# Skylarking/MARL

Hardware: NVIDIA B200
Metric: QMIX learner episode-samples/sec (2s3z shape) (higher is better)
Workload: dtype f32

## Files before the change

### marl_b200/csrc/common.cuh

```cuda
#pragma once
#include <cuda_runtime.h>
#include <stdint.h>

#define MARL_H 64
#define MARL_G (3 * MARL_H)

#define MARL_OK 0
#define MARL_EINVAL (-1)

#define MARL_LAUNCH_CHECK()                                   \
    do {                                                      \
        cudaError_t e__ = cudaGetLastError();                 \
        if (e__ != cudaSuccess) return (int)e__;              \
    } while (0)

#include <cstdlib>
#include <utility>

namespace marl {

constexpr int kNumSMs = 148;

__device__ __forceinline__ void pdl_wait() { asm volatile("griddepcontrol.wait;" ::: "memory"); }
__device__ __forceinline__ void pdl_trigger() { asm volatile("griddepcontrol.launch_dependents;" ::: "memory"); }
// ... 22 lines not shown
    return cudaLaunchKernelEx(&cfg, kern, KArgs(std::forward<Args>(args))...);
}
inline int& linear_prio() { static int v = 0; return v; }
struct LinearPrio {
    int keep;
    explicit LinearPrio(int p) : keep(linear_prio()) { linear_prio() = p; }
    ~LinearPrio() { linear_prio() = keep; }
};
template <class... KArgs, class... Args>
inline cudaError_t launch_pdl(void (*kern)(KArgs...), dim3 grid, dim3 block, size_t smem, cudaStream_t st, Args&&... args) {
    return launch_pdl_prio(0, kern, grid, block, smem, st, std::forward<Args>(args)...);
}

__device__ __forceinline__ float warp_sum(float v) {
#pragma unroll
    for (int o = 16; o > 0; o >>= 1) v += __shfl_xor_sync(0xffffffffu, v, o);
    return v;
}

__device__ __forceinline__ void cp_async16(void* smem, const void* gmem) {
    const unsigned s = (unsigned)__cvta_generic_to_shared(smem);
    asm volatile("cp.async.cg.shared.global [%0], [%1], 16;\n" ::"r"(s), "l"(gmem));
}
__device__ __forceinline__ void cp_async_commit() { asm volatile("cp.async.commit_group;\n" ::); }
template <int N>
__device__ __forceinline__ void cp_async_wait() { asm volatile("cp.async.wait_group %0;\n" ::"n"(N)); }

__device__ __forceinline__ float sigmoidf_acc(float x) { return 1.0f / (1.0f + expf(-x)); }

struct LinOperand {
    const float* x;   int ldx;  int K1;
    const float* x2;  int ldx2; int K2;
    int x2_shift;
    int x2_period;
    int onehot_mod;
    long long x_bs, x2_bs;
    int onehot_z;
};

__device__ __forceinline__ float lin_load(const LinOperand& a, int z, int m, int k) {
    if (k < a.K1) return __ldg(a.x + (long long)z * a.x_bs + (long long)m * a.ldx + k);
    k -= a.K1;
    if (k < a.K2) {
        int mm = m;
        if (a.x2_shift) {
            if ((m % a.x2_period) < a.x2_shift) return 0.0f;
// ... 12 lines not shown
```

### marl_b200/csrc/qmix.cu

```cuda
#include "linear.h"
#include "forkjoin.h"
#include "../../include/marl_b200.h"
#include "profile.h"
#include "tgemm.h"

#ifdef MARL_MIX_TRACE
__device__ long long* g_mix_trace_ptr = nullptr;
#define MIX_SEL_STAMP(tag)                                                                                      \
    do {                                                                                                        \
        if (threadIdx.x == 0 && (blockIdx.x == 0 || blockIdx.x == 300) && g_mix_trace_ptr) {                     \
            long long* t__ = g_mix_trace_ptr + (blockIdx.x ? 512 : 0);                                           \
            long long now__; asm volatile("mov.u64 %0, %%globaltimer;" : "=l"(now__));                           \
            const int n__ = (int)t__[510]; if (n__ < 60) { t__[2 * n__] = (tag); t__[2 * n__ + 1] = now__; t__[510] = n__ + 1; } \
        }                                                                                                       \
    } while (0)
#endif
#include "select.cuh"

namespace marl {

constexpr int E = MARL_QMIX_EMBED;
#ifndef MARL_QMIX_WARPS
#define MARL_QMIX_WARPS 8
#endif
constexpr int kQmixWarps = MARL_QMIX_WARPS;
constexpr int kQmixCtasPerSm = 32 / kQmixWarps;
constexpr int kQmixMaxAgents = 64;

enum { QMIX_FWD = 0, QMIX_BWD = 1, QMIX_TD = 2 };

struct QmixMixArgs {
    int M, N, A, mode;
    const float* hy;  const float* q;  const float* wb2;  const float* bb2;
    const float* hy_t; const float* q_t; const float* wb2_t; const float* bb2_t;
    const float* r; const float* term; const float* padded; float gamma;
    const float* dq_tot_in;
    float* q_tot; float* q_tot_t;
    float* dhy;
    float* dq_small;
    const long long* u; float* dq_dense;
    const float* fc2_w; float* dhext;
    SelectArgs sel;
    float* g_wb2; float* g_bb2; float* scalars;
    long long* trace;
};
#ifdef MARL_MIX_TRACE
#define MIX_STAMP(tag) MIX_SEL_STAMP(tag)
#else
#define MIX_STAMP(tag) do { } while (0)
#endif

__device__ __forceinline__ float qmix_forward_lane(const float* __restrict__ y, const float* __restrict__ q, int N,
                                                   float wb2e, float bb2, int lane, float& pre, float& hid,
                                                   float& w2raw, float& hb2) {
    float acc = y[N * E + lane];
#pragma unroll 4
    for (int n = 0; n < N; ++n) acc = fmaf(q[n], fabsf(y[n * E + lane]), acc);
    pre = acc;
    hid = acc > 0.0f ? acc : (expf(acc) - 1.0f);
    w2raw = y[N * E + E + lane];
    hb2 = y[N * E + 2 * E + lane];
    float part = hid * fabsf(w2raw) + fmaxf(hb2, 0.0f) * wb2e;
    return warp_sum(part) + bb2;
}

__global__ void __launch_bounds__(kQmixWarps * 32, kQmixCtasPerSm) qmix_mix_kernel(QmixMixArgs a) {
#ifdef MARL_MIX_TRACE
    if (threadIdx.x == 0 && (blockIdx.x == 0 || blockIdx.x == 300)) g_mix_trace_ptr = a.trace;
#endif
    MIX_STAMP(0);
    pdl_enter();
    MIX_STAMP(1);
    __shared__ float sdq[kQmixWarps][kQmixMaxAgents];
    __shared__ float sred[kQmixWarps][E + 1];
    __shared__ float ssel[kQmixWarps][2][kQmixMaxAgents];
    extern __shared__ __align__(16) float ssel_dyn[];
    const float* heads = nullptr;
    if (a.sel.q && a.sel.heads) {
        const int m_first = blockIdx.x * kQmixWarps + (threadIdx.x >> 5);
        if (m_first < a.M)
            warp_stage_hidden_async(a.sel, m_first, a.N, a.A, threadIdx.x & 31, ssel_dyn + (threadIdx.x >> 5) * select_warp_floats(a.N, a.A, true));
        float* h = ssel_dyn + kQmixWarps * select_warp_floats(a.N, a.A, true);
        stage_heads(a.sel, a.A, h);
        heads = h;
        __syncthreads();
    }
    bool prestaged = a.sel.q && a.sel.heads;
    MIX_STAMP(2);
    const int lane = threadIdx.x & 31, warp = threadIdx.x >> 5;
    const int N = a.N, C = N * E + 3 * E;
    const float wb2e = a.wb2[lane], bb2 = a.bb2[0];
    float wb2te = 0.f, bb2t = 0.f;
    if (a.mode == QMIX_TD) { wb2te = a.wb2_t[lane]; bb2t = a.bb2_t[0]; }
    float acc_wb2 = 0.f, acc_bb2 = 0.f, acc_sq = 0.f, acc_mask = 0.f;
    for (int m = blockIdx.x * kQmixWarps + warp; m < a.M; m += gridDim.x * kQmixWarps) {
        const float* __restrict__ y = a.hy + (long long)m * C;
        const float* q = a.q + (long long)m * N;
        const float* qt = a.q_t + (long long)m * N;
        if (a.sel.q) {
            warp_select(a.sel, m, N, a.A, lane, ssel_dyn + warp * select_warp_floats(N, a.A, a.sel.heads), ssel[warp][0], ssel[warp][1], heads, prestaged);
            prestaged = false;
            q = ssel[warp][0]; qt = ssel[warp][1];
        }
        MIX_STAMP(3);
        float pre, hid, w2raw, hb2;
        const float tot = qmix_forward_lane(y, q, N, wb2e, bb2, lane, pre, hid, w2raw, hb2);
        if (lane == 0 && a.q_tot) a.q_tot[m] = tot;
        MIX_STAMP(4);
        if (a.mode == QMIX_FWD) continue;
        float G;
        if (a.mode == QMIX_TD) {
            float p2, h2, w2t, hbt;
            const float tot_t = qmix_forward_lane(a.hy_t + (long long)m * C, qt, N, wb2te, bb2t,
                                                  lane, p2, h2, w2t, hbt);
            if (lane == 0 && a.q_tot_t) a.q_tot_t[m] = tot_t;
            const float mask = 1.0f - a.padded[m];
            const float yt = a.r[m] + a.gamma * tot_t * (1.0f - a.term[m]);
            const float d = mask * (yt - tot);
            acc_sq += d * d; acc_mask += mask;
            G = -2.0f * mask * d;
        } else {
            G = a.dq_tot_in[m];
        }
        MIX_STAMP(5);
        float* __restrict__ dy = a.dhy + (long long)m * C;
        const float dpre = G * fabsf(w2raw) * (pre > 0.0f ? 1.0f : (hid + 1.0f));
        const float sgn2 = (w2raw > 0.0f) ? 1.0f : (w2raw < 0.0f ? -1.0f : 0.0f);
        dy[N * E + lane] = dpre;
        dy[N * E + E + lane] = G * hid * sgn2;
        dy[N * E + 2 * E + lane] = (hb2 > 0.0f) ? G * wb2e : 0.0f;
        acc_wb2 += G * fmaxf(hb2, 0.0f);
        acc_bb2 += G;
#pragma unroll 4
        for (int n = 0; n < N; ++n) {
            const float w1raw = y[n * E + lane];
            const float sgn1 = (w1raw > 0.0f) ? 1.0f : (w1raw < 0.0f ? -1.0f : 0.0f);
            dy[n * E + lane] = dpre * q[n] * sgn1;
            const float dqn = warp_sum(dpre * fabsf(w1raw));
            if (lane == 0) sdq[warp][n] = dqn;
        }
        __syncwarp();
        MIX_STAMP(6);
        if (a.dq_small)
            for (int n = lane; n < N; n += 32) a.dq_small[(long long)m * N + n] = sdq[warp][n];
        if (a.dq_dense) {
            const int A = a.A;
            for (int i = lane; i < N * A; i += 32) {
                const int n = i / A, c = i - n * A;
                a.dq_dense[(long long)m * N * A + i] = (c == (int)a.u[(long long)m * N + n]) ? sdq[warp][n] : 0.0f;
            }
        }
        if (a.dhext) warp_dhext(a.fc2_w, a.u, m, N, lane, sdq[warp], a.dhext);
        __syncwarp();
        MIX_STAMP(7);
    }
    if (a.mode == QMIX_FWD) return;
    sred[warp][lane] = acc_wb2;
    if (lane == 0) sred[warp][E] = acc_bb2;
    __syncthreads();
    if (warp == 0) {
        float v = 0.f, b = 0.f;
        for (int w = 0; w < kQmixWarps; ++w) { v += sred[w][lane]; b += sred[w][E]; }
        if (a.g_wb2) atomicAdd(a.g_wb2 + lane, v);
        if (lane == 0 && a.g_bb2) atomicAdd(a.g_bb2, b);
    }
    if (a.mode == QMIX_TD) {
        __syncthreads();
        if (lane == 0) { sred[warp][0] = acc_sq; sred[warp][1] = acc_mask; }
        __syncthreads();
        if (threadIdx.x == 0) {
            float v = 0.f, b = 0.f;
            for (int w = 0; w < kQmixWarps; ++w) { v += sred[w][0]; b += sred[w][1]; }
            atomicAdd(a.scalars, v); atomicAdd(a.scalars + 1, b);
        }
    }
    MIX_STAMP(8);
}

static int hyper_fwd(int M, int N, int S, const marl_qmix_params* p, const float* s, float* hy, cudaStream_t st) {
    LinearFwd f{};
    f.in = plain_operand(s, S, S);
    f.w = p->wcat; f.ldw = S; f.bias = p->bcat;
    f.y = hy; f.ldy = N * E + 3 * E; f.M = M; f.N = N * E + 3 * E; f.batch = 1;
    return linear_fwd(f, st);
}

static int hyper_wgrad(int M, int N, int S, const float* s, const float* dhy, const marl_qmix_grads* g, cudaStream_t st) {
    LinearWgrad w{};
    w.dy = dhy; w.lddy = N * E + 3 * E; w.in = plain_operand(s, S, S);
    w.dw = g->wcat; w.ldw = S; w.db = g->bcat; w.M = M; w.N = N * E + 3 * E; w.batch = 1;
    return linear_wgrad(w, st);
}

static int hyper2_fwd(int M, int N, int S, const marl_qmix_hyper2* p, const float* s, float* h, float* hy, cudaStream_t st) {
    const int hh = p->hh, C = N * E + 3 * E;
    int rc;
    LinearFwd f{};
    f.in = plain_operand(s, S, S); f.w = p->w_in; f.ldw = S; f.bias = p->b_in;
    f.y = h; f.ldy = 2 * hh; f.M = M; f.N = 2 * hh; f.relu = 1; f.batch = 1;
// ... 24 lines not shown
    w.dy = dhy + N * E; w.lddy = C; w.in = plain_operand(s, S, S); w.dw = g->w_b1; w.ldw = S; w.db = g->b_b1; w.M = M; w.N = E; w.batch = 1;
    if ((rc = linear_wgrad(w, st))) return rc;
    w.dy = dhy + N * E + 2 * E; w.dw = g->w_b20; w.db = g->b_b20;
    if ((rc = linear_wgrad(w, st))) return rc;
    LinearWgrad o1{};
    o1.dy = dhy; o1.lddy = C; o1.in = plain_operand(h, 2 * hh, hh); o1.dw = g->w1_out; o1.ldw = hh; o1.db = g->b1_out; o1.M = M; o1.N = N * E; o1.batch = 1;
    if ((rc = linear_wgrad(o1, st))) return rc;
    LinearWgrad o2{};
    o2.dy = dhy + N * E + E; o2.lddy = C; o2.in = plain_operand(h + hh, 2 * hh, hh); o2.dw = g->w2_out; o2.ldw = hh; o2.db = g->b2_out; o2.M = M; o2.N = E; o2.batch = 1;
    if ((rc = linear_wgrad(o2, st))) return rc;
    LinearDgrad d1{};
    d1.dy = dhy; d1.lddy = C; d1.w = p->w1_out; d1.ldw = hh; d1.dx = dh; d1.lddx = 2 * hh; d1.relu_src = h; d1.ldrs = 2 * hh;
    d1.M = M; d1.N = N * E; d1.K = hh; d1.batch = 1;
    if ((rc = linear_dgrad(d1, st))) return rc;
    LinearDgrad d2{};
    d2.dy = dhy + N * E + E; d2.lddy = C; d2.w = p->w2_out; d2.ldw = hh; d2.dx = dh + hh; d2.lddx = 2 * hh; d2.relu_src = h + hh; d2.ldrs = 2 * hh;
    d2.M = M; d2.N = E; d2.K = hh; d2.batch = 1;
    if ((rc = linear_dgrad(d2, st))) return rc;
    LinearWgrad i{};
    i.dy = dh; i.lddy = 2 * hh; i.in = plain_operand(s, S, S); i.dw = g->w_in; i.ldw = S; i.db = g->b_in; i.M = M; i.N = 2 * hh; i.batch = 1;
    return linear_wgrad(i, st);
}

static int mix_grid(int M) {
    int blocks = (M + kQmixWarps - 1) / kQmixWarps;
    return blocks < 1 ? 1 : (blocks > kQmixCtasPerSm * kNumSMs ? kQmixCtasPerSm * kNumSMs : blocks);
}

}

using namespace marl;

static bool qmix_params_ok(const marl_qmix_params* p) { return p && p->wcat && p->bcat && p->wb2 && p->bb2; }

extern "C" int marl_qmix_fwd(int M, int N, int S, const marl_qmix_params* p, const float* q, const float* s, float* hy,
                             float* q_tot, void* stream) {
    if (M < 0 || N < 1 || N > kQmixMaxAgents || S < 1 || !qmix_params_ok(p) || !q || !s || !hy || !q_tot) return MARL_EINVAL;
    if (M == 0) return MARL_OK;
    cudaStream_t st = (cudaStream_t)stream;
    int rc = hyper_fwd(M, N, S, p, s, hy, st);
    if (rc) return rc;
    QmixMixArgs a{};
    a.M = M; a.N = N; a.mode = QMIX_FWD; a.hy = hy; a.q = q; a.wb2 = p->wb2; a.bb2 = p->bb2; a.q_tot = q_tot;
    { ProfScope ps_("qmix_mix_kernel", st); launch_pdl(qmix_mix_kernel, dim3(mix_grid(M)), dim3(kQmixWarps * 32), 0, st, a); }
    MARL_LAUNCH_CHECK();
    return MARL_OK;
}

extern "C" int marl_qmix_bwd(int M, int N, int S, const marl_qmix_params* p, const float* q, const float* s,
                             const float* hy, const float* dq_tot, float* dhy, float* dq, const marl_qmix_grads* g,
                             void* stream) {
    if (M < 0 || N < 1 || N > kQmixMaxAgents || S < 1 || !qmix_params_ok(p) || !q || !s || !hy || !dq_tot || !dhy || !g)
        return MARL_EINVAL;
    if (M == 0) return MARL_OK;
    cudaStream_t st = (cudaStream_t)stream;
    QmixMixArgs a{};
    a.M = M; a.N = N; a.mode = QMIX_BWD; a.hy = hy; a.q = q; a.wb2 = p->wb2; a.bb2 = p->bb2;
    a.dq_tot_in = dq_tot; a.dhy = dhy; a.dq_small = dq; a.g_wb2 = g->wb2; a.g_bb2 = g->bb2;
    { ProfScope ps_("qmix_mix_kernel", st); launch_pdl(qmix_mix_kernel, dim3(mix_grid(M)), dim3(kQmixWarps * 32), 0, st, a); }
    MARL_LAUNCH_CHECK();
    return hyper_wgrad(M, N, S, s, dhy, g, st);
}

extern "C" int marl_qmix_td_fwd_bwd(const marl_dims* d, const marl_qmix_params* p, const marl_qmix_params* pt,
                                    const float* s, const float* s_next, float* q_chosen, float* q_tc,
                                    const long long* u, const float* r, const float* terminated, const float* padded,
                                    float gamma, float* hy, float* hy_target, float* dhy, float* q_tot, float* q_tot_target,
                                    float* dq, const marl_qmix_grads* g, float* scalars, int flags, const float* fc2_w,
                                    float* dhext, const marl_select_fused* sel, void* stream) {
    if (!d || !p || !pt || !p->wb2 || !p->bb2 || !pt->wb2 || !pt->bb2 || !s || !s_next || !q_chosen || !q_tc || !r ||
        !terminated || !padded || !hy || !hy_target || !dhy || !g || !scalars)
        return MARL_EINVAL;
    if (!(flags & 1) && (!p->wcat || !p->bcat || !pt->wcat || !pt->bcat)) return MARL_EINVAL;
    if (!(flags & 2) && (!g->wcat || !g->bcat)) return MARL_EINVAL;
    if ((dq || dhext || sel) && !u) return MARL_EINVAL;
    if (sel && !select_ok(sel)) return MARL_EINVAL;
    if (dhext && (!fc2_w || ((uintptr_t)fc2_w & 7) || ((uintptr_t)dhext & 7))) return MARL_EINVAL;
    if (d->N < 1 || d->N > kQmixMaxAgents || d->S < 1) return MARL_EINVAL;
    const int M = d->B * d->L;
    if (M <= 0) return MARL_OK;
    cudaStream_t st = (cudaStream_t)stream;
    pdl_scope((long long)M * d->N);
    int rc;
    if (!(flags & 1)) {
        ForkJoin fj(st, 2);
        if ((rc = hyper_fwd(M, d->N, d->S, p, s, hy, fj.lane(0)))) return rc;
        if ((rc = hyper_fwd(M, d->N, d->S, pt, s_next, hy_target, fj.lane(1)))) return rc;
        fj.join();
    }
    QmixMixArgs a{};
    a.M = M; a.N = d->N; a.A = d->A; a.mode = QMIX_TD;
    a.hy = hy; a.q = q_chosen; a.wb2 = p->wb2; a.bb2 = p->bb2;
    a.hy_t = hy_target; a.q_t = q_tc; a.wb2_t = pt->wb2; a.bb2_t = pt->bb2;
    a.r = r; a.term = terminated; a.padded = padded; a.gamma = gamma;
    a.q_tot = q_tot; a.q_tot_t = q_tot_target; a.dhy = dhy; a.u = u; a.dq_dense = dq;
    a.fc2_w = fc2_w; a.dhext = dhext;
    if (sel) a.sel = select_args(sel, u, q_chosen, q_tc);
    a.g_wb2 = g->wb2; a.g_bb2 = g->bb2; a.scalars = scalars;
    a.trace = trace_buffer();
    const size_t dyn = sel ? select_smem(kQmixWarps, d->N, d->A, sel->hidden_evals != nullptr) : 0;
    if (dyn > kSelectSmemMax) return MARL_EINVAL;
    if (dyn > 40 * 1024) {
        static bool attr_set = false;
        if (!attr_set) { cudaFuncSetAttribute(qmix_mix_kernel, cudaFuncAttributeMaxDynamicSharedMemorySize, (int)kSelectSmemMax); attr_set = true; }
    }
    { ProfScope ps_("qmix_mix_kernel", st); launch_pdl(qmix_mix_kernel, dim3(mix_grid(M)), dim3(kQmixWarps * 32), dyn, st, a); }
    MARL_LAUNCH_CHECK();
    if (flags & 2) return MARL_OK;
    return hyper_wgrad(M, d->N, d->S, s, dhy, g, st);
}

extern "C" int marl_qmix_mix_fwd(int M, int N, const marl_qmix_params* p, const float* q, const float* hy, float* q_tot,
                                 void* stream) {
    if (M < 0 || N < 1 || N > kQmixMaxAgents || !p || !p->wb2 || !p->bb2 || !q || !hy || !q_tot) return MARL_EINVAL;
    if (M == 0) return MARL_OK;
    cudaStream_t st = (cudaStream_t)stream;
    QmixMixArgs a{};
    a.M = M; a.N = N; a.mode = QMIX_FWD; a.hy = hy; a.q = q; a.wb2 = p->wb2; a.bb2 = p->bb2; a.q_tot = q_tot;
    { ProfScope ps_("qmix_mix_kernel", st); launch_pdl(qmix_mix_kernel, dim3(mix_grid(M)), dim3(kQmixWarps * 32), 0, st, a); }
    MARL_LAUNCH_CHECK();
    return MARL_OK;
}

extern "C" int marl_qmix_mix_bwd(int M, int N, const marl_qmix_params* p, const float* q, const float* hy,
                                 const float* dq_tot, float* dhy, float* dq, const marl_qmix_grads* g, void* stream) {
    if (M < 0 || N < 1 || N > kQmixMaxAgents || !p || !p->wb2 || !p->bb2 || !q || !hy || !dq_tot || !dhy || !g) return MARL_EINVAL;
    if (M == 0) return MARL_OK;
    cudaStream_t st = (cudaStream_t)stream;
    QmixMixArgs a{};
    a.M = M; a.N = N; a.mode = QMIX_BWD; a.hy = hy; a.q = q; a.wb2 = p->wb2; a.bb2 = p->bb2;
    a.dq_tot_in = dq_tot; a.dhy = dhy; a.dq_small = dq; a.g_wb2 = g->wb2; a.g_bb2 = g->bb2;
    { ProfScope ps_("qmix_mix_kernel", st); launch_pdl(qmix_mix_kernel, dim3(mix_grid(M)), dim3(kQmixWarps * 32), 0, st, a); }
    MARL_LAUNCH_CHECK();
    return MARL_OK;
}

static bool hyper2_ok(const marl_qmix_hyper2* p) {
    return p && p->hh > 0 && p->w_in && p->b_in && p->w1_out && p->b1_out && p->w2_out && p->b2_out && p->w_b1 && p->b_b1 &&
           p->w_b20 && p->b_b20;
}

extern "C" int marl_qmix_hyper2_fwd(int M, int N, int S, const marl_qmix_hyper2* p, const float* s, float* h, float* hy,
                                    void* stream) {
    if (M < 0 || N < 1 || N > kQmixMaxAgents || S < 1 || !hyper2_ok(p) || !s || !h || !hy) return MARL_EINVAL;
    if (M == 0) return MARL_OK;
    return hyper2_fwd(M, N, S, p, s, h, hy, (cudaStream_t)stream);
}

extern "C" int marl_qmix_hyper2_bwd(int M, int N, int S, const marl_qmix_hyper2* p, const float* s, const float* h,
                                    const float* dhy, float* dh, const marl_qmix_hyper2_grads* g, void* stream) {
    if (M < 0 || N < 1 || N > kQmixMaxAgents || S < 1 || !hyper2_ok(p) || !s || !h || !dhy || !dh || !g || !g->w_in ||
        !g->b_in || !g->w1_out || !g->b1_out || !g->w2_out || !g->b2_out || !g->w_b1 || !g->b_b1 || !g->w_b20 || !g->b_b20)
        return MARL_EINVAL;
    if (M == 0) return MARL_OK;
    return hyper2_bwd(M, N, S, p, s, h, dhy, dh, g, (cudaStream_t)stream);
}

extern "C" int marl_qmix_hyper_fwd(int M, int N, int S, const marl_qmix_params* p, const float* s, float* hy, void* stream) {
    if (M < 0 || N < 1 || N > kQmixMaxAgents || S < 1 || !qmix_params_ok(p) || !s || !hy) return MARL_EINVAL;
    if (M == 0) return MARL_OK;
    pdl_scope((long long)M * N);
    return hyper_fwd(M, N, S, p, s, hy, (cudaStream_t)stream);
}

extern "C" int marl_qmix_hyper_wgrad(int M, int N, int S, const float* s, const float* dhy, const marl_qmix_grads* g,
                                     void* stream) {
    if (M < 0 || N < 1 || N > kQmixMaxAgents || S < 1 || !s || !dhy || !g || !g->wcat || !g->bcat) return MARL_EINVAL;
    if (M == 0) return MARL_OK;
    pdl_scope((long long)M * N);
    return hyper_wgrad(M, N, S, s, dhy, g, (cudaStream_t)stream);
}

extern "C" int marl_select_fits(int qmix, int N, int A, int heads) {
    if (N <= 0 || A <= 0) return 0;
    return marl::select_smem(qmix ? marl::kQmixWarps : 8, N, A, heads != 0) <= marl::kSelectSmemMax ? 1 : 0;
}
```

### marl_b200/csrc/select.cuh

```cuda
#pragma once
#include "common.cuh"
#include "../../include/marl_b200.h"

#ifndef MIX_SEL_STAMP
#define MIX_SEL_STAMP(tag) do { } while (0)
#endif

namespace marl {

constexpr float kNegBig = -9999999.0f;

struct SelectArgs {
    float* q; float* qn; float* qt; const float* avail_next; const long long* u;
    float* q_out; float* qt_out; long long* a_star;
    int heads;
    const float* h_e; const float* h_t; const float* h_n;
    const float* w2; const float* b2; const float* w2t; const float* b2t;
};

inline SelectArgs select_args(const marl_select_fused* s, const long long* u, float* q_chosen, float* q_tc) {
    SelectArgs a{};
    a.q = s->q_evals; a.qn = s->q_evals_next; a.qt = s->q_targets; a.avail_next = s->avail_u_next; a.u = u;
    a.q_out = q_chosen; a.qt_out = q_tc; a.a_star = s->a_star;
    a.heads = s->hidden_evals != nullptr;
    a.h_e = s->hidden_evals; a.h_t = s->hidden_targets; a.h_n = s->hidden_evals_next;
    a.w2 = s->fc2_w; a.b2 = s->fc2_b; a.w2t = s->fc2_w_target; a.b2t = s->fc2_b_target;
    return a;
}
inline bool select_ok(const marl_select_fused* s) {
// ... 34 lines not shown
    for (int i = threadIdx.x; i < A; i += blockDim.x) {
        dst[2 * A * kHeadLd + i] = s.b2[i];
        dst[2 * A * kHeadLd + A + i] = s.b2t[i];
    }
}

__device__ __forceinline__ void warp_stage_hidden_async(const SelectArgs& s, long long m, int N, int A, int lane, float* stage) {
    constexpr int Q = MARL_H / 4, LQ = kHeadLd / 4;
    const int NA = N * A;
    float4* she = (float4*)(stage + ((3 * NA + 3) & ~3));
    float4* sht = she + N * LQ;
    float4* shn = sht + N * LQ;
    const float4* ge = (const float4*)(s.h_e + m * N * MARL_H);
    const float4* gt = (const float4*)(s.h_t + m * N * MARL_H);
    const float4* gn = s.h_n ? (const float4*)(s.h_n + m * N * MARL_H) : ge;
    for (int i = lane; i < N * Q; i += 32) {
        const int n = i / Q, k = i - n * Q;
        cp_async16(she + n * LQ + k, ge + i); cp_async16(sht + n * LQ + k, gt + i); cp_async16(shn + n * LQ + k, gn + i);
    }
    cp_async_commit();
}

__device__ __forceinline__ void warp_select(const SelectArgs& s, long long m, int N, int A, int lane, float* stage,
                                            float* qc, float* tc, const float* heads, bool prestaged = false) {
    const int NA = N * A;
    const long long o = m * NA;
    float* sn = stage;
    float* st = stage + NA;
    float* se = stage + 2 * NA;
    if (s.heads) {
        constexpr int Q = MARL_H / 4, LQ = kHeadLd / 4;
        float4* she = (float4*)(stage + ((3 * NA + 3) & ~3));
        float4* sht = she + N * LQ;
        float4* shn = sht + N * LQ;
        if (!prestaged) warp_stage_hidden_async(s, m, N, A, lane, stage);
#if MARL_HEADS_MMA
        float av_pre[2];
#pragma unroll
        for (int it = 0; it < 2; ++it) av_pre[it] = lane + 32 * it < NA ? s.avail_next[o + lane + 32 * it] : 1.0f;
#endif
        cp_async_wait<0>();
        __syncwarp();
        MIX_SEL_STAMP(31);
#if MARL_HEADS_MMA
        {
            const int R3 = 3 * N, g = lane >> 2, t = lane & 3;
            const float* hrows = (const float*)she;
            const float* bias = heads + 2 * A * kHeadLd;
            for (int m0 = 0; m0 < R3; m0 += 16) {
                const int ra = m0 + g, rb = m0 + g + 8;
                const float* pa = hrows + min(ra, R3 - 1) * kHeadLd + t;
                const float* pb = hrows + min(rb, R3 - 1) * kHeadLd + t;
                const bool has_t = m0 < 2 * N && m0 + 16 > N, has_e = m0 < N || m0 + 16 > 2 * N;
                for (int set = 0; set < 2; ++set) {
                    if (set ? !has_t : !has_e) continue;
                    for (int c0 = 0; c0 < A; c0 += 16) {
                        const bool two = c0 + 8 < A;
                        const float* w0 = heads + (set * A + min(c0 + g, A - 1)) * kHeadLd + t;
                        const float* w1 = heads + (set * A + min(c0 + 8 + g, A - 1)) * kHeadLd + t;
                        float am[2][4] = {}, ac[2][4] = {};
#pragma unroll
                        for (int ks = 0; ks < MARL_H / 8; ++ks) {
                            uint32_t ah[4], al[4];
                            head_split(pa[8 * ks], ah[0], al[0]); head_split(pb[8 * ks], ah[1], al[1]);
                            head_split(pa[8 * ks + 4], ah[2], al[2]); head_split(pb[8 * ks + 4], ah[3], al[3]);
#pragma unroll
                            for (int jj = 0; jj < 2; ++jj) {
                                if (jj && !two) continue;
                                const float* w = jj ? w1 : w0;
                                uint32_t bh[2], bl[2];
                                head_split(w[8 * ks], bh[0], bl[0]); head_split(w[8 * ks + 4], bh[1], bl[1]);
                                head_mma(ac[jj], al, bh); head_mma(ac[jj], ah, bl); head_mma(am[jj], ah, bh);
                            }
                        }
                        MIX_SEL_STAMP(33);
#pragma unroll
                        for (int h = 0; h < 2; ++h) {
                            const int r = h ? rb : ra;
                            if (r >= R3) continue;
                            const int slab = r / N, n = r - slab * N;
                            if ((slab == 1) != (set == 1)) continue;
                            float* dst = (slab == 0 ? se : slab == 1 ? st : sn) + n * A;
#pragma unroll
                            for (int jj = 0; jj < 2; ++jj)
#pragma unroll
                                for (int e = 0; e < 2; ++e) {
                                    const int a = c0 + 8 * jj + 2 * t + e;
                                    if (a < A) dst[a] = (am[jj][2 * h + e] + ac[jj][2 * h + e]) + bias[set * A + a];
                                }
                        }
                    }
                }
            }
            __syncwarp();
            MIX_SEL_STAMP(34);
            for (int i = lane, it = 0; i < NA; i += 32, ++it) {
                const bool off = (it < 2 ? av_pre[it & 1] : s.avail_next[o + i]) == 0.0f;
                s.q[o + i] = se[i];
                const float qt = off ? kNegBig : st[i];
                s.qt[o + i] = qt; st[i] = qt;
                if (s.qn) { const float qn = sn[i]; s.qn[o + i] = qn; sn[i] = off ? kNegBig : qn; }
            }
        }
#else
        const int A2 = (A + 1) >> 1;
        for (int i = lane; i < N * A2; i += 32) {
            const int n = i / A2, ap = i - n * A2, a0 = 2 * ap, a1 = a0 + 1 < A ? a0 + 1 : a0;
            const float4* w0 = (const float4*)(heads + a0 * kHeadLd);
            const float4* w1 = (const float4*)(heads + a1 * kHeadLd);
            const float4* v0 = (const float4*)(heads + (A + a0) * kHeadLd);
            const float4* v1 = (const float4*)(heads + (A + a1) * kHeadLd);
            const float4* he = she + n * LQ;
            const float4* ht = sht + n * LQ;
            const float4* hn = shn + n * LQ;
            const float4 z4 = make_float4(0.f, 0.f, 0.f, 0.f);
            float4 ce0 = z4, cn0 = z4, ct0 = z4, ce1 = z4, cn1 = z4, ct1 = z4;
#pragma unroll 2
            for (int k = 0; k < Q; ++k) {
// ... 14 lines not shown
                const float4 ce = h ? ce1 : ce0, cn = h ? cn1 : cn0, ct = h ? ct1 : ct0;
                float qe = (ce.x + ce.y) + (ce.z + ce.w), qn = (cn.x + cn.y) + (cn.z + cn.w), qt = (ct.x + ct.y) + (ct.z + ct.w);
                const float be = heads[2 * A * kHeadLd + a], bt = heads[2 * A * kHeadLd + A + a];
                qe += be; qn += be; qt += bt;
                const int j = n * A + a;
                const bool off = s.avail_next[o + j] == 0.0f;
                if (off) qt = kNegBig;
                s.q[o + j] = qe; s.qt[o + j] = qt;
                se[j] = qe; st[j] = qt;
                if (s.qn) { s.qn[o + j] = qn; sn[j] = off ? kNegBig : qn; }
            }
        }
#endif
    } else {
        for (int i = lane; i < NA; i += 32) {
            const bool off = s.avail_next[o + i] == 0.0f;
            float v = s.qt[o + i];
            if (off) { v = kNegBig; s.qt[o + i] = v; }
            st[i] = v;
            if (s.qn) sn[i] = off ? kNegBig : s.qn[o + i];
        }
    }
    __syncwarp();
    MIX_SEL_STAMP(32);
    for (int n = lane; n < N; n += 32) {
        const long long i = m * N + n;
        const float c = s.heads ? se[n * A + (int)s.u[i]] : s.q[i * A + s.u[i]];
        int best = 0;
        float tmax = 0.f, tsel = 0.f;
        if (s.qn) {
            float bv = 0.f;
            for (int a = 0; a < A; ++a) {
                const float v = sn[n * A + a];
                if (a == 0 || v > bv) { bv = v; best = a; }
            }
        }
        for (int a = 0; a < A; ++a) {
            const float v = st[n * A + a];
            if (a == 0 || v > tmax) tmax = v;
            if (a == best) tsel = v;
        }
        const float t = s.qn ? tsel : tmax;
        qc[n] = c; tc[n] = t;
        s.q_out[i] = c; s.qt_out[i] = t;
        if (s.a_star) s.a_star[i] = s.qn ? best : -1;
    }
    __syncwarp();
// ... 14 lines not shown
```

Before: 106,700.

## Restructure QMIX mix kernel to stage multi-sample blocks in shared memory

Replaces the per-warp, one-sample-at-a-time mix kernel with a block that handles S samples at once. All inputs (hypernet outputs, q values, availability masks, actions, rewards and head weights) are bulk-staged into shared memory with cp.async, and the action-head MMA runs cooperatively across the block. S and the grid size are picked at launch time from M and a shared-memory budget so that roughly one block lands per SM. The aim is fewer global memory round trips and better load batching, at the cost of extra __syncthreads, large dynamic shared memory, and occupancy that now depends on M.

```diff
diff --git a/marl_b200/csrc/common.cuh b/marl_b200/csrc/common.cuh
--- a/marl_b200/csrc/common.cuh
+++ b/marl_b200/csrc/common.cuh
@@ -68,6 +68,14 @@
     const unsigned s = (unsigned)__cvta_generic_to_shared(smem);
     asm volatile("cp.async.cg.shared.global [%0], [%1], 16;\n" ::"r"(s), "l"(gmem));
 }
+__device__ __forceinline__ void cp_async8(void* smem, const void* gmem) {
+    const unsigned s = (unsigned)__cvta_generic_to_shared(smem);
+    asm volatile("cp.async.ca.shared.global [%0], [%1], 8;\n" ::"r"(s), "l"(gmem));
+}
+__device__ __forceinline__ void cp_async4(void* smem, const void* gmem) {
+    const unsigned s = (unsigned)__cvta_generic_to_shared(smem);
+    asm volatile("cp.async.ca.shared.global [%0], [%1], 4;\n" ::"r"(s), "l"(gmem));
+}
 __device__ __forceinline__ void cp_async_commit() { asm volatile("cp.async.commit_group;\n" ::); }
 template <int N>
 __device__ __forceinline__ void cp_async_wait() { asm volatile("cp.async.wait_group %0;\n" ::"n"(N)); }
diff --git a/marl_b200/csrc/qmix.cu b/marl_b200/csrc/qmix.cu
--- a/marl_b200/csrc/qmix.cu
+++ b/marl_b200/csrc/qmix.cu
@@ -1,36 +1,25 @@
+#include <algorithm>
 #include "linear.h"
 #include "forkjoin.h"
 #include "../../include/marl_b200.h"
 #include "profile.h"
 #include "tgemm.h"
-
-#ifdef MARL_MIX_TRACE
-__device__ long long* g_mix_trace_ptr = nullptr;
-#define MIX_SEL_STAMP(tag)                                                                                      \
-    do {                                                                                                        \
-        if (threadIdx.x == 0 && (blockIdx.x == 0 || blockIdx.x == 300) && g_mix_trace_ptr) {                     \
-            long long* t__ = g_mix_trace_ptr + (blockIdx.x ? 512 : 0);                                           \
-            long long now__; asm volatile("mov.u64 %0, %%globaltimer;" : "=l"(now__));                           \
-            const int n__ = (int)t__[510]; if (n__ < 60) { t__[2 * n__] = (tag); t__[2 * n__ + 1] = now__; t__[510] = n__ + 1; } \
-        }                                                                                                       \
-    } while (0)
-#endif
 #include "select.cuh"
 
 namespace marl {
 
 constexpr int E = MARL_QMIX_EMBED;
-#ifndef MARL_QMIX_WARPS
-#define MARL_QMIX_WARPS 8
-#endif
-constexpr int kQmixWarps = MARL_QMIX_WARPS;
-constexpr int kQmixCtasPerSm = 32 / kQmixWarps;
 constexpr int kQmixMaxAgents = 64;
+constexpr int kMixMaxSamples = 28;
+constexpr size_t kMixStaticSmem = kMixMaxSamples * (E + 1) * sizeof(float);
+constexpr size_t kMixSmemMax = 220 * 1024;
+constexpr size_t kSmemPerSm = 228 * 1024, kSmemPerCta = 1024;
 
 enum { QMIX_FWD = 0, QMIX_BWD = 1, QMIX_TD = 2 };
 
 struct QmixMixArgs {
     int M, N, A, mode;
+    int S;
     const float* hy;  const float* q;  const float* wb2;  const float* bb2;
     const float* hy_t; const float* q_t; const float* wb2_t; const float* bb2_t;
     const float* r; const float* term; const float* padded; float gamma;
@@ -45,10 +34,58 @@
     long long* trace;
 };
 #ifdef MARL_MIX_TRACE
-#define MIX_STAMP(tag) MIX_SEL_STAMP(tag)
+#define MIX_STAMP(tag)                                                                                          \
+    do {                                                                                                        \
+        if (threadIdx.x == 0 && (blockIdx.x == 0 || blockIdx.x == 100) && a.trace) {                             \
+            long long* t__ = a.trace + (blockIdx.x ? 512 : 0);                                                   \
+            long long now__; asm volatile("mov.u64 %0, %%globaltimer;" : "=l"(now__));                           \
+            const int n__ = (int)t__[510]; if (n__ < 60) { t__[2 * n__] = (tag); t__[2 * n__ + 1] = now__; t__[510] = n__ + 1; } \
+        }                                                                                                       \
+    } while (0)
 #else
 #define MIX_STAMP(tag) do { } while (0)
 #endif
+
+struct MixLayout { int heads, hid, y, yt, slab, av, qc, tc, dq, u, r, term, pad, g, total; };
+__host__ __device__ inline int round4(int x) { return (x + 3) & ~3; }
+__host__ __device__ inline MixLayout mix_layout(int S, int N, int A, bool sel, bool heads, bool td) {
+    const int C = N * E + 3 * E, SN = S * N;
+    MixLayout l;
+    int o = 0;
+    l.heads = o; o += heads ? round4(2 * A * kHeadLd + 2 * A) : 0;
+    l.hid = o;   o += heads ? 3 * SN * kHeadLd : 0;
+    l.y = o;     o += S * C;
+    l.yt = o;    o += td ? S * C : 0;
+    l.slab = o;  o += sel ? round4(3 * SN * A) : 0;
+    l.av = o;    o += sel ? round4(SN * A) : 0;
+    l.qc = o;    o += round4(SN);
+    l.tc = o;    o += round4(SN);
+    l.dq = o;    o += round4(SN);
+    l.u = o;     o += td ? 2 * round4(SN) : 0;
+    l.r = o;     o += round4(S);
+    l.term = o;  o += round4(S);
+    l.pad = o;   o += round4(S);
+    l.g = o;     o += round4(S);
+    l.total = o;
+    return l;
+}
+
+__device__ __forceinline__ void block_fetch(float* dst, const float* src, int n) {
+    if (((((uintptr_t)dst | (uintptr_t)src) & 15) | (n & 3)) == 0)
+        for (int i = threadIdx.x; i < (n >> 2); i += blockDim.x) cp_async16(dst + 4 * i, src + 4 * i);
+    else
+        for (int i = threadIdx.x; i < n; i += blockDim.x) cp_async4(dst + i, src + i);
+}
+__device__ __forceinline__ void block_fetch_i64(long long* dst, const long long* src, int n) {
+    for (int i = threadIdx.x; i < n; i += blockDim.x) cp_async8(dst + i, src + i);
+}
+__device__ __forceinline__ void block_fetch_rows(float* dst, const float* src, int rows) {
+    constexpr int Q = MARL_H / 4;
+    for (int i = threadIdx.x; i < rows * Q; i += blockDim.x) {
+        const int r = i / Q, k = i - r * Q;
+        cp_async16(dst + r * kHeadLd + 4 * k, src + 4 * i);
+    }
+}
 
 __device__ __forceinline__ float qmix_forward_lane(const float* __restrict__ y, const float* __restrict__ q, int N,
                                                    float wb2e, float bb2, int lane, float& pre, float& hid,
@@ -64,95 +101,223 @@
     return warp_sum(part) + bb2;
 }
 
-__global__ void __launch_bounds__(kQmixWarps * 32, kQmixCtasPerSm) qmix_mix_kernel(QmixMixArgs a) {
-#ifdef MARL_MIX_TRACE
-    if (threadIdx.x == 0 && (blockIdx.x == 0 || blockIdx.x == 300)) g_mix_trace_ptr = a.trace;
-#endif
+__device__ __forceinline__ void block_heads(const float* hw, const float* hid, float* slab, int SN, int A, bool has_n,
+                                            int warp, int nwarps, int lane) {
+    const float* bias = hw + 2 * A * kHeadLd;
+    const int R0 = (has_n ? 2 : 1) * SN, T0 = (R0 + 15) >> 4, T1 = (SN + 15) >> 4, CP = (A + 15) >> 4;
+    const int g = lane >> 2, t = lane & 3;
+    for (int it = warp; it < (T0 + T1) * CP; it += nwarps) {
+        const int tile = it / CP, c0 = (it - tile * CP) * 16, set = tile >= T0;
+        const int hi = set ? 3 * SN : R0;
+        const int ra = (set ? 2 * SN + (tile - T0) * 16 : tile * 16) + g, rb = ra + 8;
+        const float* pa = hid + min(ra, hi - 1) * kHeadLd + t;
+        const float* pb = hid + min(rb, hi - 1) * kHeadLd + t;
+        const bool two = c0 + 8 < A;
+        const float* w0 = hw + (set * A + min(c0 + g, A - 1)) * kHeadLd + t;
+        const float* w1 = hw + (set * A + min(c0 + 8 + g, A - 1)) * kHeadLd + t;
+        float am[2][4] = {}, ac[2][4] = {};
+#pragma unroll
+        for (int ks = 0; ks < MARL_H / 8; ++ks) {
+            uint32_t ah[4], al[4];
+            head_split(pa[8 * ks], ah[0], al[0]); head_split(pb[8 * ks], ah[1], al[1]);
+            head_split(pa[8 * ks + 4], ah[2], al[2]); head_split(pb[8 * ks + 4], ah[3], al[3]);
+#pragma unroll
+            for (int jj = 0; jj < 2; ++jj) {
+                if (jj && !two) continue;
+                const float* w = jj ? w1 : w0;
+                uint32_t bh[2], bl[2];
+                head_split(w[8 * ks], bh[0], bl[0]); head_split(w[8 * ks + 4], bh[1], bl[1]);
+                head_mma(ac[jj], al, bh); head_mma(ac[jj], ah, bl); head_mma(am[jj], ah, bh);
+            }
+        }
+#pragma unroll
+        for (int h = 0; h < 2; ++h) {
+            const int r = h ? rb : ra;
+            if (r >= hi) continue;
+            float* dst = slab + r * A;
+#pragma unroll
+            for (int jj = 0; jj < 2; ++jj)
+#pragma unroll
+                for (int e = 0; e < 2; ++e) {
+                    const int c = c0 + 8 * jj + 2 * t + e;
+                    if (c < A) dst[c] = (am[jj][2 * h + e] + ac[jj][2 * h + e]) + bias[set * A + c];
+                }
+        }
+    }
+}
+
+__global__ void __launch_bounds__(kMixMaxSamples * 32, 1) qmix_mix_kernel(QmixMixArgs a) {
+    extern __shared__ __align__(16) float sm[];
+    __shared__ float sred[kMixMaxSamples][E + 1];
+    const int lane = threadIdx.x & 31, warp = threadIdx.x >> 5, nwarps = blockDim.x >> 5;
+    const int N = a.N, A = a.A, S = a.S, C = N * E + 3 * E, SN = S * N, NA = N * A;
+    const bool td = a.mode == QMIX_TD, sel = a.sel.q != nullptr, heads = sel && a.sel.heads;
+    const MixLayout l = mix_layout(S, N, A, sel, heads, td);
     MIX_STAMP(0);
+    if (heads) {
+        block_fetch_rows(sm + l.heads, a.sel.w2, A);
+        block_fetch_rows(sm + l.heads + A * kHeadLd, a.sel.w2t, A);
+        block_fetch(sm + l.heads + 2 * A * kHeadLd, a.sel.b2, A);
+        block_fetch(sm + l.heads + 2 * A * kHeadLd + A, a.sel.b2t, A);
+    }
     pdl_enter();
     MIX_STAMP(1);
-    __shared__ float sdq[kQmixWarps][kQmixMaxAgents];
-    __shared__ float sred[kQmixWarps][E + 1];
-    __shared__ float ssel[kQmixWarps][2][kQmixMaxAgents];
-    extern __shared__ __align__(16) float ssel_dyn[];
-    const float* heads = nullptr;
-    if (a.sel.q && a.sel.heads) {
-        const int m_first = blockIdx.x * kQmixWarps + (threadIdx.x >> 5);
-        if (m_first < a.M)
-            warp_stage_hidden_async(a.sel, m_first, a.N, a.A, threadIdx.x & 31, ssel_dyn + (threadIdx.x >> 5) * select_warp_floats(a.N, a.A, true));
-        float* h = ssel_dyn + kQmixWarps * select_warp_floats(a.N, a.A, true);
-        stage_heads(a.sel, a.A, h);
-        heads = h;
-        __syncthreads();
-    }
-    bool prestaged = a.sel.q && a.sel.heads;
-    MIX_STAMP(2);
-    const int lane = threadIdx.x & 31, warp = threadIdx.x >> 5;
-    const int N = a.N, C = N * E + 3 * E;
     const float wb2e = a.wb2[lane], bb2 = a.bb2[0];
     float wb2te = 0.f, bb2t = 0.f;
-    if (a.mode == QMIX_TD) { wb2te = a.wb2_t[lane]; bb2t = a.bb2_t[0]; }
+    if (td) { wb2te = a.wb2_t[lane]; bb2t = a.bb2_t[0]; }
+    const bool w2_staged = heads && a.fc2_w == a.sel.w2;
+    const float* w2 = w2_staged ? sm + l.heads : a.fc2_w;
+    const int w2_ld = w2_staged ? kHeadLd : MARL_H;
     float acc_wb2 = 0.f, acc_bb2 = 0.f, acc_sq = 0.f, acc_mask = 0.f;
-    for (int m = blockIdx.x * kQmixWarps + warp; m < a.M; m += gridDim.x * kQmixWarps) {
-        const float* __restrict__ y = a.hy + (long long)m * C;
-        const float* q = a.q + (long long)m * N;
-        const float* qt = a.q_t + (long long)m * N;
-        if (a.sel.q) {
-            warp_select(a.sel, m, N, a.A, lane, ssel_dyn + warp * select_warp_floats(N, a.A, a.sel.heads), ssel[warp][0], ssel[warp][1], heads, prestaged);
-            prestaged = false;
-            q = ssel[warp][0]; qt = ssel[warp][1];
-        }
+    for (int blk = blockIdx.x; (long long)blk * S < a.M; blk += gridDim.x) {
+        const long long m0 = (long long)blk * S;
+        const int Sv = min(S, a.M - (int)m0);
+        if (heads) {
+            block_fetch_rows(sm + l.hid, a.sel.h_e + m0 * N * MARL_H, Sv * N);
+            if (a.sel.h_n) block_fetch_rows(sm + l.hid + SN * kHeadLd, a.sel.h_n + m0 * N * MARL_H, Sv * N);
+            block_fetch_rows(sm + l.hid + 2 * SN * kHeadLd, a.sel.h_t + m0 * N * MARL_H, Sv * N);
+        } else if (sel) {
+            block_fetch(sm + l.slab, a.sel.q + m0 * NA, Sv * NA);
+            if (a.sel.qn) block_fetch(sm + l.slab + SN * A, a.sel.qn + m0 * NA, Sv * NA);
+            block_fetch(sm + l.slab + 2 * SN * A, a.sel.qt + m0 * NA, Sv * NA);
+        }
+        cp_async_commit();
+        block_fetch(sm + l.y, a.hy + m0 * C, Sv * C);
+        if (td) block_fetch(sm + l.yt, a.hy_t + m0 * C, Sv * C);
+        if (sel) {
+            block_fetch(sm + l.av, a.sel.avail_next + m0 * NA, Sv * NA);
+        } else {
+            block_fetch(sm + l.qc, a.q + m0 * N, Sv * N);
+            if (td) block_fetch(sm + l.tc, a.q_t + m0 * N, Sv * N);
+        }
+        if (td) {
+            if (a.u) block_fetch_i64((long long*)(sm + l.u), a.u + m0 * N, Sv * N);
+            block_fetch(sm + l.r, a.r + m0, Sv);
+            block_fetch(sm + l.term, a.term + m0, Sv);
+            block_fetch(sm + l.pad, a.padded + m0, Sv);
+        } else if (a.mode == QMIX_BWD) {
+            block_fetch(sm + l.g, a.dq_tot_in + m0, Sv);
+        }
+        cp_async_commit();
+        float* se = sm + l.slab;
+        float* sn = se + SN * A;
+        float* st = sn + SN * A;
+        if (heads) {
+            cp_async_wait<1>();
+            __syncthreads();
+            MIX_STAMP(2);
+            block_heads(sm + l.heads, sm + l.hid, se, SN, A, a.sel.h_n != nullptr, warp, nwarps, lane);
+        }
+        cp_async_wait<0>();
+        __syncthreads();
         MIX_STAMP(3);
-        float pre, hid, w2raw, hb2;
-        const float tot = qmix_forward_lane(y, q, N, wb2e, bb2, lane, pre, hid, w2raw, hb2);
-        if (lane == 0 && a.q_tot) a.q_tot[m] = tot;
-        MIX_STAMP(4);
-        if (a.mode == QMIX_FWD) continue;
-        float G;
-        if (a.mode == QMIX_TD) {
-            float p2, h2, w2t, hbt;
-            const float tot_t = qmix_forward_lane(a.hy_t + (long long)m * C, qt, N, wb2te, bb2t,
-                                                  lane, p2, h2, w2t, hbt);
-            if (lane == 0 && a.q_tot_t) a.q_tot_t[m] = tot_t;
-            const float mask = 1.0f - a.padded[m];
-            const float yt = a.r[m] + a.gamma * tot_t * (1.0f - a.term[m]);
-            const float d = mask * (yt - tot);
-            acc_sq += d * d; acc_mask += mask;
-            G = -2.0f * mask * d;
-        } else {
-            G = a.dq_tot_in[m];
-        }
-        MIX_STAMP(5);
-        float* __restrict__ dy = a.dhy + (long long)m * C;
-        const float dpre = G * fabsf(w2raw) * (pre > 0.0f ? 1.0f : (hid + 1.0f));
-        const float sgn2 = (w2raw > 0.0f) ? 1.0f : (w2raw < 0.0f ? -1.0f : 0.0f);
-        dy[N * E + lane] = dpre;
-        dy[N * E + E + lane] = G * hid * sgn2;
-        dy[N * E + 2 * E + lane] = (hb2 > 0.0f) ? G * wb2e : 0.0f;
-        acc_wb2 += G * fmaxf(hb2, 0.0f);
-        acc_bb2 += G;
+        if (sel) {
+            const float* av = sm + l.av;
+            const long long o0 = m0 * NA;
+            for (int i = threadIdx.x; i < Sv * NA; i += blockDim.x) {
+                const bool off = av[i] == 0.0f;
+                if (heads) {
+                    a.sel.q[o0 + i] = se[i];
+                    const float qt = off ? kNegBig : st[i];
+                    a.sel.qt[o0 + i] = qt; st[i] = qt;
+                    if (a.sel.qn) { const float qn = sn[i]; a.sel.qn[o0 + i] = qn; sn[i] = off ? kNegBig : qn; }
+                } else if (off) {
+                    st[i] = kNegBig; a.sel.qt[o0 + i] = kNegBig;
+                    if (a.sel.qn) sn[i] = kNegBig;
+                }
+            }
+            __syncthreads();
+            MIX_STAMP(4);
+        }
+        if (warp < Sv) {
+            const int s = warp;
+            const long long m = m0 + s;
+            float* qc = sm + l.qc + s * N;
+            float* tc = sm + l.tc + s * N;
+            float* sdq = sm + l.dq + s * N;
+            const long long* us = (const long long*)(sm + l.u) + s * N;
+            if (sel) {
+                for (int n = lane; n < N; n += 32) {
+                    const int j = (s * N + n) * A;
+                    const float c = se[j + (int)us[n]];
+                    int best = 0;
+                    float tmax = 0.f, tsel = 0.f;
+                    if (a.sel.qn) {
+                        float bv = 0.f;
+                        for (int c2 = 0; c2 < A; ++c2) {
+                            const float v = sn[j + c2];
+                            if (c2 == 0 || v > bv) { bv = v; best = c2; }
+                        }
+                    }
+                    for (int c2 = 0; c2 < A; ++c2) {
+                        const float v = st[j + c2];
+                        if (c2 == 0 || v > tmax) tmax = v;
+                        if (c2 == best) tsel = v;
+                    }
+                    const float t = a.sel.qn ? tsel : tmax;
+                    qc[n] = c; tc[n] = t;
+                    a.sel.q_out[m * N + n] = c; a.sel.qt_out[m * N + n] = t;
+                    if (a.sel.a_star) a.sel.a_star[m * N + n] = a.sel.qn ? best : -1;
+                }
+                __syncwarp();
+                MIX_STAMP(5);
+            }
+            const float* y = sm + l.y + s * C;
+            float pre, hid, w2raw, hb2;
+            const float tot = qmix_forward_lane(y, qc, N, wb2e, bb2, lane, pre, hid, w2raw, hb2);
+            if (lane == 0 && a.q_tot) a.q_tot[m] = tot;
+            MIX_STAMP(6);
+            if (a.mode != QMIX_FWD) {
+                float G;
+                if (td) {
+                    float p2, h2, w2t, hbt;
+                    const float tot_t = qmix_forward_lane(sm + l.yt + s * C, tc, N, wb2te, bb2t, lane, p2, h2, w2t, hbt);
+                    if (lane == 0 && a.q_tot_t) a.q_tot_t[m] = tot_t;
+                    const float mask = 1.0f - sm[l.pad + s];
+                    const float yt = sm[l.r + s] + a.gamma * tot_t * (1.0f - sm[l.term + s]);
+                    const float d = mask * (yt - tot);
+                    acc_sq += d * d; acc_mask += mask;
+                    G = -2.0f * mask * d;
+                } else {
+                    G = sm[l.g + s];
+                }
+                MIX_STAMP(7);
+                float* __restrict__ dy = a.dhy + m * C;
+                const float dpre = G * fabsf(w2raw) * (pre > 0.0f ? 1.0f : (hid + 1.0f));
+                const float sgn2 = (w2raw > 0.0f) ? 1.0f : (w2raw < 0.0f ? -1.0f : 0.0f);
+                dy[N * E + lane] = dpre;
+                dy[N * E + E + lane] = G * hid * sgn2;
+                dy[N * E + 2 * E + lane] = (hb2 > 0.0f) ? G * wb2e : 0.0f;
+                acc_wb2 += G * fmaxf(hb2, 0.0f);
+                acc_bb2 += G;
 #pragma unroll 4
-        for (int n = 0; n < N; ++n) {
-            const float w1raw = y[n * E + lane];
-            const float sgn1 = (w1raw > 0.0f) ? 1.0f : (w1raw < 0.0f ? -1.0f : 0.0f);
-            dy[n * E + lane] = dpre * q[n] * sgn1;
-            const float dqn = warp_sum(dpre * fabsf(w1raw));
-            if (lane == 0) sdq[warp][n] = dqn;
-        }
-        __syncwarp();
-        MIX_STAMP(6);
-        if (a.dq_small)
-            for (int n = lane; n < N; n += 32) a.dq_small[(long long)m * N + n] = sdq[warp][n];
-        if (a.dq_dense) {
-            const int A = a.A;
-            for (int i = lane; i < N * A; i += 32) {
-                const int n = i / A, c = i - n * A;
-                a.dq_dense[(long long)m * N * A + i] = (c == (int)a.u[(long long)m * N + n]) ? sdq[warp][n] : 0.0f;
+                for (int n = 0; n < N; ++n) {
+                    const float w1raw = y[n * E + lane];
+                    const float sgn1 = (w1raw > 0.0f) ? 1.0f : (w1raw < 0.0f ? -1.0f : 0.0f);
+                    dy[n * E + lane] = dpre * qc[n] * sgn1;
+                    const float dqn = warp_sum(dpre * fabsf(w1raw));
+                    if (lane == 0) sdq[n] = dqn;
+                }
+                __syncwarp();
+                MIX_STAMP(8);
+                if (a.dq_small)
+                    for (int n = lane; n < N; n += 32) a.dq_small[m * N + n] = sdq[n];
+                if (a.dq_dense)
+                    for (int i = lane; i < NA; i += 32) {
+                        const int n = i / A, c = i - n * A;
+                        a.dq_dense[m * NA + i] = (c == (int)us[n]) ? sdq[n] : 0.0f;
+                    }
+                if (a.dhext)
+#pragma unroll 4
+                    for (int n = 0; n < N; ++n) {
+                        const float gn = sdq[n];
+                        const float2 w = ((const float2*)(w2 + us[n] * w2_ld))[lane];
+                        ((float2*)(a.dhext + (m * N + n) * MARL_H))[lane] = make_float2(gn * w.x, gn * w.y);
+                    }
+                MIX_STAMP(9);
             }
         }
-        if (a.dhext) warp_dhext(a.fc2_w, a.u, m, N, lane, sdq[warp], a.dhext);
-        __syncwarp();
-        MIX_STAMP(7);
+        __syncthreads();
     }
     if (a.mode == QMIX_FWD) return;
     sred[warp][lane] = acc_wb2;
@@ -160,21 +325,21 @@
     __syncthreads();
     if (warp == 0) {
         float v = 0.f, b = 0.f;
-        for (int w = 0; w < kQmixWarps; ++w) { v += sred[w][lane]; b += sred[w][E]; }
+        for (int w = 0; w < nwarps; ++w) { v += sred[w][lane]; b += sred[w][E]; }
         if (a.g_wb2) atomicAdd(a.g_wb2 + lane, v);
         if (lane == 0 && a.g_bb2) atomicAdd(a.g_bb2, b);
     }
-    if (a.mode == QMIX_TD) {
+    if (td) {
         __syncthreads();
         if (lane == 0) { sred[warp][0] = acc_sq; sred[warp][1] = acc_mask; }
         __syncthreads();
         if (threadIdx.x == 0) {
             float v = 0.f, b = 0.f;
-            for (int w = 0; w < kQmixWarps; ++w) { v += sred[w][0]; b += sred[w][1]; }
+            for (int w = 0; w < nwarps; ++w) { v += sred[w][0]; b += sred[w][1]; }
             atomicAdd(a.scalars, v); atomicAdd(a.scalars + 1, b);
         }
     }
-    MIX_STAMP(8);
+    MIX_STAMP(10);
 }
 
 static int hyper_fwd(int M, int N, int S, const marl_qmix_params* p, const float* s, float* hy, cudaStream_t st) {
@@ -245,9 +410,23 @@
     return linear_wgrad(i, st);
 }
 
-static int mix_grid(int M) {
-    int blocks = (M + kQmixWarps - 1) / kQmixWarps;
-    return blocks < 1 ? 1 : (blocks > kQmixCtasPerSm * kNumSMs ? kQmixCtasPerSm * kNumSMs : blocks);
+static int launch_mix(QmixMixArgs& a, cudaStream_t st) {
+    const bool td = a.mode == QMIX_TD, sel = a.sel.q != nullptr, heads = sel && a.sel.heads;
+    const auto bytes = [&](int S) { return (size_t)mix_layout(S, a.N, a.A, sel, heads, td).total * sizeof(float); };
+    int S = (a.M + kNumSMs - 1) / kNumSMs, per_sm = 1;
+    if (S > kMixMaxSamples) { S = kMixMaxSamples / 2; per_sm = 2; }
+    const size_t cap = std::min(kMixSmemMax, kSmemPerSm / per_sm - kSmemPerCta - kMixStaticSmem);
+    while (S > 1 && bytes(S) > cap) --S;
+    const size_t smem = bytes(S);
+    if (smem > cap) return MARL_EINVAL;
+    const int fit = std::max(1, std::min((int)(kSmemPerSm / (smem + kSmemPerCta + kMixStaticSmem)), kMixMaxSamples / S));
+    const int blocks = (a.M + S - 1) / S, grid = std::min(blocks, fit * kNumSMs);
+    a.S = S;
+    static bool attr_set = false;
+    if (!attr_set) { cudaFuncSetAttribute(qmix_mix_kernel, cudaFuncAttributeMaxDynamicSharedMemorySize, (int)kMixSmemMax); attr_set = true; }
+    { ProfScope ps_("qmix_mix_kernel", st); launch_pdl(qmix_mix_kernel, dim3(grid), dim3(S * 32), smem, st, a); }
+    MARL_LAUNCH_CHECK();
+    return MARL_OK;
 }
 
 }
@@ -265,9 +444,7 @@
     if (rc) return rc;
     QmixMixArgs a{};
     a.M = M; a.N = N; a.mode = QMIX_FWD; a.hy = hy; a.q = q; a.wb2 = p->wb2; a.bb2 = p->bb2; a.q_tot = q_tot;
-    { ProfScope ps_("qmix_mix_kernel", st); launch_pdl(qmix_mix_kernel, dim3(mix_grid(M)), dim3(kQmixWarps * 32), 0, st, a); }
-    MARL_LAUNCH_CHECK();
-    return MARL_OK;
+    return launch_mix(a, st);
 }
 
 extern "C" int marl_qmix_bwd(int M, int N, int S, const marl_qmix_params* p, const float* q, const float* s,
@@ -280,8 +457,8 @@
     QmixMixArgs a{};
     a.M = M; a.N = N; a.mode = QMIX_BWD; a.hy = hy; a.q = q; a.wb2 = p->wb2; a.bb2 = p->bb2;
     a.dq_tot_in = dq_tot; a.dhy = dhy; a.dq_small = dq; a.g_wb2 = g->wb2; a.g_bb2 = g->bb2;
-    { ProfScope ps_("qmix_mix_kernel", st); launch_pdl(qmix_mix_kernel, dim3(mix_grid(M)), dim3(kQmixWarps * 32), 0, st, a); }
-    MARL_LAUNCH_CHECK();
+    const int rc = launch_mix(a, st);
+    if (rc) return rc;
     return hyper_wgrad(M, N, S, s, dhy, g, st);
 }
 
@@ -321,14 +498,7 @@
     if (sel) a.sel = select_args(sel, u, q_chosen, q_tc);
     a.g_wb2 = g->wb2; a.g_bb2 = g->bb2; a.scalars = scalars;
     a.trace = trace_buffer();
-    const size_t dyn = sel ? select_smem(kQmixWarps, d->N, d->A, sel->hidden_evals != nullptr) : 0;
-    if (dyn > kSelectSmemMax) return MARL_EINVAL;
-    if (dyn > 40 * 1024) {
-        static bool attr_set = false;
-        if (!attr_set) { cudaFuncSetAttribute(qmix_mix_kernel, cudaFuncAttributeMaxDynamicSharedMemorySize, (int)kSelectSmemMax); attr_set = true; }
-    }
-    { ProfScope ps_("qmix_mix_kernel", st); launch_pdl(qmix_mix_kernel, dim3(mix_grid(M)), dim3(kQmixWarps * 32), dyn, st, a); }
-    MARL_LAUNCH_CHECK();
+    if ((rc = launch_mix(a, st))) return rc;
     if (flags & 2) return MARL_OK;
     return hyper_wgrad(M, d->N, d->S, s, dhy, g, st);
 }
@@ -340,9 +510,7 @@
     cudaStream_t st = (cudaStream_t)stream;
     QmixMixArgs a{};
     a.M = M; a.N = N; a.mode = QMIX_FWD; a.hy = hy; a.q = q; a.wb2 = p->wb2; a.bb2 = p->bb2; a.q_tot = q_tot;
-    { ProfScope ps_("qmix_mix_kernel", st); launch_pdl(qmix_mix_kernel, dim3(mix_grid(M)), dim3(kQmixWarps * 32), 0, st, a); }
-    MARL_LAUNCH_CHECK();
-    return MARL_OK;
+    return launch_mix(a, st);
 }
 
 extern "C" int marl_qmix_mix_bwd(int M, int N, const marl_qmix_params* p, const float* q, const float* hy,
@@ -353,9 +521,7 @@
     QmixMixArgs a{};
     a.M = M; a.N = N; a.mode = QMIX_BWD; a.hy = hy; a.q = q; a.wb2 = p->wb2; a.bb2 = p->bb2;
     a.dq_tot_in = dq_tot; a.dhy = dhy; a.dq_small = dq; a.g_wb2 = g->wb2; a.g_bb2 = g->bb2;
-    { ProfScope ps_("qmix_mix_kernel", st); launch_pdl(qmix_mix_kernel, dim3(mix_grid(M)), dim3(kQmixWarps * 32), 0, st, a); }
-    MARL_LAUNCH_CHECK();
-    return MARL_OK;
+    return launch_mix(a, st);
 }
 
 static bool hyper2_ok(const marl_qmix_hyper2* p) {
@@ -396,5 +562,6 @@
 
 extern "C" int marl_select_fits(int qmix, int N, int A, int heads) {
     if (N <= 0 || A <= 0) return 0;
-    return marl::select_smem(qmix ? marl::kQmixWarps : 8, N, A, heads != 0) <= marl::kSelectSmemMax ? 1 : 0;
-}
+    (void)qmix;
+    return marl::select_smem(8, N, A, heads != 0) <= marl::kSelectSmemMax ? 1 : 0;
+}
diff --git a/marl_b200/csrc/select.cuh b/marl_b200/csrc/select.cuh
--- a/marl_b200/csrc/select.cuh
+++ b/marl_b200/csrc/select.cuh
@@ -1,10 +1,6 @@
 #pragma once
 #include "common.cuh"
 #include "../../include/marl_b200.h"
-
-#ifndef MIX_SEL_STAMP
-#define MIX_SEL_STAMP(tag) do { } while (0)
-#endif
 
 namespace marl {
 
@@ -85,7 +81,7 @@
 }
 
 __device__ __forceinline__ void warp_select(const SelectArgs& s, long long m, int N, int A, int lane, float* stage,
-                                            float* qc, float* tc, const float* heads, bool prestaged = false) {
+                                            float* qc, float* tc, const float* heads) {
     const int NA = N * A;
     const long long o = m * NA;
     float* sn = stage;
@@ -96,7 +92,7 @@
         float4* she = (float4*)(stage + ((3 * NA + 3) & ~3));
         float4* sht = she + N * LQ;
         float4* shn = sht + N * LQ;
-        if (!prestaged) warp_stage_hidden_async(s, m, N, A, lane, stage);
+        warp_stage_hidden_async(s, m, N, A, lane, stage);
 #if MARL_HEADS_MMA
         float av_pre[2];
 #pragma unroll
@@ -104,7 +100,6 @@
 #endif
         cp_async_wait<0>();
         __syncwarp();
-        MIX_SEL_STAMP(31);
 #if MARL_HEADS_MMA
         {
             const int R3 = 3 * N, g = lane >> 2, t = lane & 3;
@@ -136,7 +131,6 @@
                                 head_mma(ac[jj], al, bh); head_mma(ac[jj], ah, bl); head_mma(am[jj], ah, bh);
                             }
                         }
-                        MIX_SEL_STAMP(33);
 #pragma unroll
                         for (int h = 0; h < 2; ++h) {
                             const int r = h ? rb : ra;
@@ -156,7 +150,6 @@
                 }
             }
             __syncwarp();
-            MIX_SEL_STAMP(34);
             for (int i = lane, it = 0; i < NA; i += 32, ++it) {
                 const bool off = (it < 2 ? av_pre[it & 1] : s.avail_next[o + i]) == 0.0f;
                 s.q[o + i] = se[i];
@@ -217,7 +210,6 @@
         }
     }
     __syncwarp();
-    MIX_SEL_STAMP(32);
     for (int n = lane; n < N; n += 32) {
         const long long i = m * N + n;
         const float c = s.heads ? se[n * A + (int)s.u[i]] : s.q[i * A + s.u[i]];
```

Result: faster. 110,500 (median of 6 runs) (+3.5%).
